# refresh-bio/DSRC

Hardware: AMD Instinct MI355X
Metric: raw FASTQ MB/s compressed (bit-identical .dsrc) at -d3 -q2 (higher is better)
Workload: dtype u8/u16/u32 integer

## Files before the change

### dsrc_amd/csrc/k_parse.h

```cpp
#pragma once
#include "k_common.h"

typedef u64 __attribute__((aligned(1))) u64_text;

__device__ __forceinline__ u32 byte_eq8(u64 w, u64 c_rep)
{
	const u64 x = w ^ c_rep;
	const u64 y = (((x & 0x7F7F7F7F7F7F7F7Full) + 0x7F7F7F7F7F7F7F7Full) | x) | 0x7F7F7F7F7F7F7F7Full;
	return (u32)((((~y) >> 7) * 0x0102040810204080ull) >> 56);
}

struct LineBits { u64 term, crlf; };

__device__ __forceinline__ LineBits classify64(const u8* p, u64 base, u64 size)
{
	LineBits r; r.term = 0; r.crlf = 0;
	if (base >= size) return r;
	u64 lf = 0, cr = 0;
	if (base + DSRC_LANE_BYTES <= size)
	{
#pragma unroll
		for (u32 k = 0; k < DSRC_LANE_BYTES / 8; ++k)
		{
			const u64 w = *(const u64_text*)(p + base + 8 * k);
			lf |= (u64)byte_eq8(w, 0x0A0A0A0A0A0A0A0Aull) << (8 * k);
			cr |= (u64)byte_eq8(w, 0x0D0D0D0D0D0D0D0Dull) << (8 * k);
		}
	}
	else
	{
		for (u32 k = 0; base + k < size; ++k)
		{
			const u8 c = p[base + k];
			if (c == '\n') lf |= 1ull << k;
			if (c == '\r') cr |= 1ull << k;
		}
	}
	const u64 n_valid = size - base;
	const u64 valid = n_valid >= 64 ? ~0ull : ((1ull << n_valid) - 1ull);
	const bool lf_next = base + DSRC_LANE_BYTES < size && p[base + DSRC_LANE_BYTES] == '\n';
	const bool cr_prev = base > 0 && p[base - 1] == '\r';
	const u64 lf_after = (lf >> 1) | (lf_next ? 1ull << 63 : 0ull);
	const u64 cr_before = (cr << 1) | (cr_prev ? 1ull : 0ull);
	r.term = (lf | (cr & ~lf_after)) & valid;
	r.crlf = (lf & cr_before) & valid;
	return r;
}

__global__ void __launch_bounds__(WG) k_count_lines(const u8* in, const BlkDesc* desc, BlkState* st, u32* tile_cnt, DsrcParams prm)
{
	__shared__ u32 s_tot[2];
	const u32 b = blockIdx.y, tile = blockIdx.x;
	const BlkDesc d = desc[b];
	if (tile >= d.n_tiles) return;
	if (threadIdx.x < 2) s_tot[threadIdx.x] = 0;
	__syncthreads();
	const LineBits lb = classify64(in + d.in_off, (u64)tile * DSRC_TILE_BYTES + (u64)threadIdx.x * DSRC_LANE_BYTES, d.in_size);
	const u32 cnt = wave_sum((u32)__popcll(lb.term)), crlf = wave_sum((u32)__popcll(lb.crlf));
	if (lane_id() == 0) { if (cnt) atomicAdd(&s_tot[0], cnt); if (crlf) atomicAdd(&s_tot[1], crlf); }
	__syncthreads();
	if (threadIdx.x == 0)
	{
		tile_cnt[(u64)b * prm.max_tiles + tile] = s_tot[0];
		atomicAdd(&st[b].n_term, s_tot[0]);
		if (s_tot[1]) atomicAdd(&st[b].n_crlf, s_tot[1]);
	}
}

__global__ void __launch_bounds__(WG) k_scan_tiles(const BlkDesc* desc, u32* tile_cnt, DsrcParams prm)
{
	const u32 b = blockIdx.x;
	const u32 n = desc[b].n_tiles;
	u32* t = tile_cnt + (u64)b * prm.max_tiles;
	u32 carry = 0;
	for (u32 base = 0; base < n; base += blockDim.x)
	{
		const u32 i = base + threadIdx.x;
		const u32 v = i < n ? t[i] : 0;
		u32 tot;
		const u32 ex = block_excl_scan(v, &tot);
		if (i < n) t[i] = carry + ex;
		carry += tot;
	}
}

__global__ void __launch_bounds__(WG) k_index_lines(const u8* in, const BlkDesc* desc, const u32* tile_base, u32* line_start, DsrcParams prm)
{
	const u32 b = blockIdx.y, tile = blockIdx.x;
	const BlkDesc d = desc[b];
	if (tile >= d.n_tiles) return;
	const u64 base = (u64)tile * DSRC_TILE_BYTES + (u64)threadIdx.x * DSRC_LANE_BYTES;
	const LineBits lb = classify64(in + d.in_off, base, d.in_size);
	u64 mask = lb.term;
	u32 total;
	u32 rank = block_excl_scan((u32)__popcll(mask), &total) + tile_base[(u64)b * prm.max_tiles + tile];
	u32* ls = line_start + d.line_base;
	if (tile == 0 && threadIdx.x == 0) ls[0] = 0;
	while (mask)
	{
		const u32 k = (u32)__ffsll((long long)mask) - 1;
		mask &= mask - 1;
		ls[++rank] = (u32)(base + k + 1) | ((u32)((lb.crlf >> k) & 1ull) << 31);
	}
}

struct RecPools
{
	u32* title_off; u32* seq_off; u32* qual_off;
	u16* title_len; u16* len;
	u16* kept; u16* trunc;
	u32* q_off; u32* d_off;
};

#define LS_POS(x) ((x) & 0x7FFFFFFFu)
__device__ __forceinline__ void line_extent(const u32* ls, u32 n_term, u32 size, u32 i, u32* start, u32* len)
{
	if (i > n_term) { *start = size; *len = 0; return; }
	const u32 s = LS_POS(ls[i]);
	*start = s;
	if (i == n_term) { *len = size - s; return; }
	const u32 nx = ls[i + 1];
	const u32 e = LS_POS(nx) - 1 - (nx >> 31);
	*len = e - s;
}

__global__ void __launch_bounds__(WG) k_records(const u8* in, const BlkDesc* desc, BlkState* st, const u32* line_start, RecPools rp)
{
	const u32 b = blockIdx.y;
	const BlkDesc d = desc[b];
	const u32 n_term = st[b].n_term;
	const u32 r = blockIdx.x * blockDim.x + threadIdx.x;
	const u32 n_cand = (n_term + 1 + 3) / 4;
	if (r >= n_cand || r >= d.rec_cap) return;
	const u8* p = in + d.in_off;
	const u32* ls = line_start + d.line_base;
	u32 s0, l0, s1, l1, s2, l2, s3, l3;
	line_extent(ls, n_term, d.in_size, 4 * r + 0, &s0, &l0);
	line_extent(ls, n_term, d.in_size, 4 * r + 1, &s1, &l1);
	line_extent(ls, n_term, d.in_size, 4 * r + 2, &s2, &l2);
	line_extent(ls, n_term, d.in_size, 4 * r + 3, &s3, &l3);
	const bool ok = s0 < d.in_size && l0 > 0 && p[s0] == '@' && l2 > 0 && l1 == l3;
	if (!ok) atomicMin(&st[b].first_bad, r);
	if (l0 > 65535u || l1 > 65535u || l3 > 65535u) atomicOr(&st[b].err, (u32)DSRC_ERR_LONG_LINE);
	const u64 g = (u64)d.rec_base + r;
	rp.title_off[g] = s0; rp.title_len[g] = (u16)l0;
	rp.seq_off[g] = s1;   rp.len[g] = (u16)l1;
	rp.qual_off[g] = s3;
}

__device__ __forceinline__ u32 dna_index(u32 c)
{
	switch (c)
	{
	case 'A': return 0; case 'G': return 1; case 'C': return 2; case 'T': return 3; case 'N': return 4;
	case 'R': return 5; case 'W': return 6; case 'S': return 7; case 'K': return 8; case 'M': return 9;
	case 'D': return 10; case 'V': return 11; case 'H': return 12; case 'B': return 13; case 'Y': return 14;
	case 'X': return 15; case 'U': return 16; case '.': return 17; case '-': return 18;
	default: return 255;
	}
}

constexpr u32 dna_index_packed(u32 c, u64 K0, u64 K1)
{
	const u32 i = c - 'A';
	const bool lo = i < 12;
	const u64 k = lo ? K0 : K1;
	const u32 j = lo ? i : i - 12;
	const u32 sh = 5 * (j < 12 ? j : 12);
	u32 v = i < 25 ? (u32)(k >> sh) & 31u : 31u;
	v = c == '.' ? 17u : v;
	v = c == '-' ? 18u : v;
	return v == 31u ? 255u : v;
}
#define DNA_INDEX_K0 0x0fa3ff607ff509a0ull
#define DNA_INDEX_K1 0xe7997019cbfffc89ull
constexpr u32 dna_index_switch_c(u32 c)
{
	switch (c)
	{
	case 'A': return 0; case 'G': return 1; case 'C': return 2; case 'T': return 3; case 'N': return 4;
	case 'R': return 5; case 'W': return 6; case 'S': return 7; case 'K': return 8; case 'M': return 9;
	case 'D': return 10; case 'V': return 11; case 'H': return 12; case 'B': return 13; case 'Y': return 14;
	case 'X': return 15; case 'U': return 16; case '.': return 17; case '-': return 18;
	default: return 255;
	}
}
constexpr bool dna_index_same()
{
	for (u32 c = 0; c < 256; ++c) if (dna_index_packed(c, DNA_INDEX_K0, DNA_INDEX_K1) != dna_index_switch_c(c)) return false;
	return true;
}
static_assert(dna_index_same(), "dna_index: packed table differs from src/RecordsProcessor.cpp:186-206");
template <bool FAST> __device__ __forceinline__ u32 dna_index_t(u32 c) { return FAST ? dna_index_packed(c, DNA_INDEX_K0, DNA_INDEX_K1) : dna_index(c); }

__device__ __forceinline__ u32 lossy_bin(u32 q)
{
	if (q < 2) return 0; if (q < 10) return 1; if (q < 20) return 2; if (q < 25) return 3;
	if (q < 30) return 4; if (q < 35) return 5; if (q < 40) return 6; if (q < 64) return 7;
	return 255;
}

#ifndef FAST_STATS
#define FAST_STATS true
#endif
#ifndef FAST_WRITE
#define FAST_WRITE true
#endif
__device__ __forceinline__ u32 transform_base_s(u32 s, u32 qual, u32 qoff, u32 lossy, u32* sidx, bool* keep);
template <bool FAST = false>
__device__ __forceinline__ u32 transform_base(u32 base, u32 qual, u32 qoff, u32 lossy, u32* sidx, bool* keep)
{
	return transform_base_s(dna_index_t<FAST>(base), qual, qoff, lossy, sidx, keep);
}
__device__ __forceinline__ void dna_index_table(u8* lut) { for (u32 i = threadIdx.x; i < 256; i += blockDim.x) lut[i] = (u8)dna_index(i); }
__device__ __forceinline__ u32 transform_base_s(u32 s, u32 qual, u32 qoff, u32 lossy, u32* sidx, bool* keep)
{
	*sidx = s;
	u32 q;
	if (!lossy)
	{
		q = (qual - qoff) & 255u;
		if (s > 3 && q < 7) { q = (q + 128u + ((s - 2u) << 3) - 16u) & 255u; *keep = false; }
		else *keep = true;
	}
	else
	{
		q = lossy_bin((qual - qoff) & 255u);
		if (s >= 4) { q = 0; *keep = false; }
		else { if (q == 0) q = 1; *keep = true; }
	}
	return q;
}

__device__ __forceinline__ u32 block_rec_count(const BlkState& S, const BlkDesc& d)
{
	u32 n_cand = (S.n_term + 1 + 3) / 4;
	if (n_cand > d.rec_cap) n_cand = d.rec_cap;
	return S.first_bad < n_cand ? S.first_bad : n_cand;
}

__global__ void __launch_bounds__(64) k_rec_count(const BlkDesc* desc, BlkState* st, u32 n_blocks)
{
	const u32 b = blockIdx.x * blockDim.x + threadIdx.x;
	if (b < n_blocks) st[b].n_recs = block_rec_count(st[b], desc[b]);
}

__device__ __forceinline__ u32 cs_state(u32 c) { return c == 'C' ? 1u : c == 'G' ? 2u : c == 'T' ? 3u : 0u; }

__global__ void __launch_bounds__(WG) k_cs_decode(u8* in, const BlkDesc* desc, BlkState* st, RecPools rp)
{
	const u32 b = blockIdx.y;
	const BlkDesc d = desc[b];
	u8* p = in + d.in_off;
	const u32 n_recs = st[b].n_recs;
	const u32 lane = lane_id();
	const u32 waves_total = gridDim.x * (blockDim.x >> 6);
	for (u32 r = blockIdx.x * (blockDim.x >> 6) + wave_id(); r < n_recs; r += waves_total)
	{
		const u64 g = (u64)d.rec_base + r;
		const u32 len = rp.len[g], so = rp.seq_off[g];
		if (len == 0) continue;
		if (lane == 0 && p[so] != p[rp.seq_off[d.rec_base]]) atomicOr(&st[b].cs_varbegin, 1u);
		u32 state = cs_state(p[so]);
		bool bad = false;
		for (u32 j0 = 0; j0 < len; j0 += 64)
		{
			const u32 j = j0 + lane;
			const bool in_r = j < len && j >= 1;
			const u32 c = in_r ? (u32)p[so + j] - '.' : 0u;
			if (c > 5) bad = true;
			const u32 col = (in_r && c >= 2 && c <= 5) ? c - 2 : 0u;
			const u64 m0 = __ballot((col & 1u) != 0), m1 = __ballot((col & 2u) != 0);
			const u64 le = lanemask_lt() | (1ull << lane);
			const u32 mine = state ^ ((u32)__popcll(m0 & le) & 1u) ^ (((u32)__popcll(m1 & le) & 1u) << 1);
			if (in_r) p[so + j] = c < 2 ? (u8)'N' : (u8)"ACGT"[mine];
			state ^= ((u32)__popcll(m0) & 1u) ^ (((u32)__popcll(m1) & 1u) << 1);
		}
		if (bad) atomicOr(&st[b].err, (u32)DSRC_ERR_BAD_BASE);
	}
}

#define STATS_PARTS_SLOT 7
__global__ void __launch_bounds__(WG) k_prep_stats(const u8* in, const BlkDesc* desc, BlkState* st, RecPools rp, DsrcParams prm)
{
	__shared__ u32 s_qf[256];
	__shared__ u32 s_df[20];
	__shared__ u32 s_acc[8];
	__shared__ u8 s_dna[256];
	__shared__ u32 s_last;
	dna_index_table(s_dna);
	const u32 b = blockIdx.y, parts = gridDim.x;
	const BlkDesc d = desc[b];
	const u8* p = in + d.in_off;
	const u32 n_recs = block_rec_count(st[b], d);

	for (u32 i = threadIdx.x; i < 256; i += blockDim.x) s_qf[i] = 0;
	if (threadIdx.x < 20) s_df[threadIdx.x] = 0;
	if (threadIdx.x < 8) s_acc[threadIdx.x] = (threadIdx.x == 3) ? 0xFFFFFFFFu : 0u;
	__syncthreads();

	const u32 lane = lane_id();
	u32 a_rle = 0, a_th = 0, a_raw = 0, a_min = 0xFFFFFFFFu, a_max = 0, a_tag = 0, a_bad = 0;
	constexpr u32 PS_AHEAD = 3;
	const u32 wstep = (blockDim.x >> 6) * parts, w0 = blockIdx.x * (blockDim.x >> 6) + wave_id();
	u32 n_len = 0, n_so = 0, n_qo = 0, n_tl = 0, n_b[PS_AHEAD], n_q[PS_AHEAD];
#pragma unroll
	for (u32 k = 0; k < PS_AHEAD; ++k) { n_b[k] = 'A'; n_q[k] = 0; }
	auto request = [&](u64 g)
	{
		n_len = rp.len[g]; n_so = rp.seq_off[g]; n_qo = rp.qual_off[g]; n_tl = rp.title_len[g];
		const u32 last = n_len ? n_len - 1u : 0u;
#pragma unroll
		for (u32 k = 0; k < PS_AHEAD; ++k)
		{
			const u32 j = min_u32(64u * k + lane, last);
			n_b[k] = p[n_so + j]; n_q[k] = p[n_qo + j];
		}
	};
	if (w0 < n_recs) request((u64)d.rec_base + w0);
	for (u32 r = w0; r < n_recs; r += wstep)
	{
		const u64 g = (u64)d.rec_base + r;
		const u32 len = n_len, so = n_so, qo = n_qo, tl = n_tl;
		u32 c_b[PS_AHEAD], c_q[PS_AHEAD];
#pragma unroll
		for (u32 k = 0; k < PS_AHEAD; ++k) { c_b[k] = n_b[k]; c_q[k] = n_q[k]; }
		if (r + wstep < n_recs) request(g + wstep);
		u32 kept = 0, th = 0, rle = 0, carry = 255, lastq = 255;
		auto chunk = [&](const u32 j0, const u32 cb_in, const u32 cq_in)
		{
			const u32 j = j0 + lane;
			const bool in_r = j < len;
			u32 sidx = 0, q = 0; bool keep = false;
			{
				const u32 cb = in_r ? cb_in : (u32)'A', cq = in_r ? cq_in : prm.quality_offset + 40u;
				const u32 qq = transform_base_s((u32)s_dna[cb & 255u], cq, prm.quality_offset, prm.lossy, &sidx, &keep);
				if (in_r) q = qq; else { keep = false; sidx = 0; }
			}
			const bool k2 = in_r && keep;
			if (in_r && sidx >= 20) a_bad = 1;
			if (k2 && sidx < 20) atomicAdd(&s_df[sidx], 1u);
			kept += (u32)__popcll(__ballot(k2));
			const u32 prev = wave_shr1(q, carry);
			const u64 change = __ballot(in_r && q != prev);
			rle += (u32)__popcll(change);
			if (__popcll(change) <= 16)
			{
				const u64 starts = change | 1ull;
				const u64 after = (starts >> lane) >> 1;
				const u32 n_in = len - j0 < 64u ? len - j0 : 64u;
				const u32 run = after ? (u32)__ffsll((long long)after) : n_in - lane;
				if (in_r && ((starts >> lane) & 1ull)) atomicAdd(&s_qf[q], run);
			}
			else if (in_r) atomicAdd(&s_qf[q], 1u);
			const u64 m2 = __ballot(in_r && q != 2);
			if (m2) th = j0 + 63u - (u32)__clzll((long long)m2);
			carry = (u32)__builtin_amdgcn_readlane((int)q, 63);
			const u32 last_lane = (len - 1 - j0) < 64u ? (len - 1 - j0) : 63u;
			lastq = (u32)__builtin_amdgcn_readlane((int)q, (int)last_lane);
		};
#pragma unroll
		for (u32 k = 0; k < PS_AHEAD; ++k) if (64u * k < len) chunk(64u * k, c_b[k], c_q[k]);
		for (u32 j0 = 64u * PS_AHEAD; j0 < len; j0 += 64)
		{
			const u32 j = min_u32(j0 + lane, len - 1u);
			chunk(j0, (u32)p[so + j], (u32)p[qo + j]);
		}
		if (len > 0 && lastq == 2 && rle > 0) rle -= 1;
		if (lane == 0)
		{
			rp.kept[g] = (u16)kept;
			rp.trunc[g] = (u16)(th + (len > 0 ? 1u : 0u));
			a_rle += rle; a_th += th; a_raw += len; a_tag += tl;
			a_min = len < a_min ? len : a_min; a_max = len > a_max ? len : a_max;
		}
	}
	if (lane == 0)
	{
		atomicAdd(&s_acc[0], a_rle); atomicAdd(&s_acc[1], a_th); atomicAdd(&s_acc[2], a_raw);
		atomicMin(&s_acc[3], a_min); atomicMax(&s_acc[4], a_max); atomicAdd(&s_acc[5], a_tag);
	}
	if (a_bad) atomicOr(&s_acc[7], 1u);
	__syncthreads();

	BlkState* S = &st[b];
	if (parts > 1)
	{
		for (u32 i = threadIdx.x; i < 256; i += blockDim.x) if (s_qf[i]) atomicAdd(&S->q_freq[i], s_qf[i]);
		if (threadIdx.x < 20 && s_df[threadIdx.x]) atomicAdd(&S->d_freq[threadIdx.x], s_df[threadIdx.x]);
		if (threadIdx.x == 0)
		{
			atomicAdd(&S->rle_len, s_acc[0]); atomicAdd(&S->th_len, s_acc[1]); atomicAdd(&S->raw_len, s_acc[2]);
			atomicMin(&S->min_len, s_acc[3]); atomicMax(&S->max_len, s_acc[4]); atomicAdd(&S->raw_tag, s_acc[5]);
			if (s_acc[7]) atomicOr(&S->err, (u32)DSRC_ERR_BAD_BASE);
		}
		__threadfence();
		__syncthreads();
		if (threadIdx.x == 0) s_last = atomicAdd(&S->scratch[STATS_PARTS_SLOT], 1u) == parts - 1u ? 1u : 0u;
		__syncthreads();
		if (!s_last) return;
		__threadfence();
		for (u32 i = threadIdx.x; i < 256; i += blockDim.x) s_qf[i] = atomicAdd(&S->q_freq[i], 0u);
		if (threadIdx.x < 20) s_df[threadIdx.x] = atomicAdd(&S->d_freq[threadIdx.x], 0u);
		if (threadIdx.x == 0)
		{
			s_acc[0] = atomicAdd(&S->rle_len, 0u); s_acc[1] = atomicAdd(&S->th_len, 0u); s_acc[2] = atomicAdd(&S->raw_len, 0u);
			s_acc[3] = atomicAdd(&S->min_len, 0u); s_acc[4] = atomicAdd(&S->max_len, 0u); s_acc[5] = atomicAdd(&S->raw_tag, 0u);
			s_acc[7] = 0;
			S->scratch[STATS_PARTS_SLOT] = 0;
		}
		__syncthreads();
	}
	else
	{
		for (u32 i = threadIdx.x; i < 256; i += blockDim.x) S->q_freq[i] = s_qf[i];
		if (threadIdx.x < 20) S->d_freq[threadIdx.x] = s_df[threadIdx.x];
	}
	if (threadIdx.x == 0)
	{
		S->n_recs = n_recs;
		S->n_lines = S->n_term + 1;
		S->rle_len = s_acc[0]; S->th_len = s_acc[1]; S->raw_len = s_acc[2];
		S->min_len = s_acc[3]; S->max_len = s_acc[4];
		S->raw_tag = s_acc[5]; S->raw_dna = s_acc[2]; S->raw_qua = s_acc[2];
		u32 e = 0;
		if (n_recs == 0) e |= DSRC_ERR_NO_RECORDS;
		if (s_acc[7]) e |= DSRC_ERR_BAD_BASE;
		if (e) atomicOr(&S->err, e);
		u32 dc = 0, qc = 0;
		for (u32 i = 0; i < 20; ++i) S->d_sym[i] = s_df[i] ? (u8)dc++ : (u8)255;
		for (u32 i = 0; i < 256; ++i) S->q_sym[i] = s_qf[i] ? (u8)qc++ : (u8)255;
		S->d_count = dc; S->q_count = qc;
	}
}

__global__ void __launch_bounds__(WG) k_cs_reduce(const u8* in, const BlkDesc* desc, BlkState* st, RecPools rp, DsrcParams prm)
{
	const u32 b = blockIdx.y;
	BlkState* S = &st[b];
	if (S->cs_varbegin) return;
	const BlkDesc d = desc[b];
	const u32 r = blockIdx.x * blockDim.x + threadIdx.x;
	if (r >= S->n_recs) return;
	const u64 g = (u64)d.rec_base + r;
	const u32 len = rp.len[g];
	if (r == 0)
	{
		const u8* p = in + d.in_off;
		u32 first = 255, q0 = 0;
		for (u32 j = 0; j < len && first == 255; ++j)
		{
			u32 sidx; bool keep;
			const u32 q = transform_base(p[rp.seq_off[g] + j], p[rp.qual_off[g] + j], prm.quality_offset, prm.lossy, &sidx, &keep);
			if (j == 0) q0 = q;
			if (keep) first = sidx;
		}
		S->cs_seq_begin = first != 255 ? first : (len ? dna_index(p[rp.seq_off[g]]) : 0u);
		S->cs_qua_begin = q0;
		S->cs_reduced = 1;
	}
	if (rp.kept[g] < 1 || len < 2) { atomicOr(&S->err, (u32)DSRC_ERR_BAD_BASE); return; }
	rp.len[g] = (u16)(len - 1); rp.qual_off[g] += 1; rp.kept[g] -= 1;
	if (rp.trunc[g] > 0) rp.trunc[g] -= 1;
}

__global__ void __launch_bounds__(WG) k_rec_offsets(const BlkDesc* desc, BlkState* st, RecPools rp)
{
	const u32 b = blockIdx.x;
	const BlkDesc d = desc[b];
	const u32 n = st[b].n_recs;
	u32 cq = 0, cd = 0;
	for (u32 base = 0; base < n; base += blockDim.x)
	{
		const u32 r = base + threadIdx.x;
		const u64 g = (u64)d.rec_base + r;
		const u32 vq = r < n ? rp.len[g] : 0, vd = r < n ? rp.kept[g] : 0;
		u32 tq, td;
		const u32 eq = block_excl_scan(vq, &tq);
		const u32 ed = block_excl_scan(vd, &td);
		if (r < n) { rp.q_off[g] = cq + eq; rp.d_off[g] = cd + ed; }
		cq += tq; cd += td;
	}
	if (threadIdx.x == 0) { st[b].q_total = cq; st[b].d_total = cd; }
}

__global__ void __launch_bounds__(WG) k_prep_write(const u8* in, const BlkDesc* desc, const BlkState* st, RecPools rp,
												   u8* q_stream, u8* qp_stream, u8* d_stream, DsrcParams prm)
{
	__shared__ u8 s_dna[256];
	dna_index_table(s_dna);
	__syncthreads();
	const u32 b = blockIdx.y;
	const BlkDesc d = desc[b];
	const u8* p = in + d.in_off;
	const u32 n_recs = st[b].n_recs;
	const u32 lane = lane_id();
	const bool write_qp = st[b].min_len != st[b].max_len;
	const u32 red = st[b].cs_reduced;
	const u32 waves_total = gridDim.x * (blockDim.x >> 6);
	constexpr u32 PW_AHEAD = 3;
	u32 n_rlen = 0, n_so = 0, n_qo = 0, n_qoff = 0, n_doff = 0;
	auto request = [&](u64 g) { n_rlen = rp.len[g]; n_so = rp.seq_off[g]; n_qo = rp.qual_off[g]; n_qoff = rp.q_off[g]; n_doff = rp.d_off[g]; };
	const u32 r0 = blockIdx.x * (blockDim.x >> 6) + wave_id();
	if (r0 < n_recs) request((u64)d.rec_base + r0);
	for (u32 r = r0; r < n_recs; r += waves_total)
	{
		const u64 g = (u64)d.rec_base + r;
		const u32 rlen = n_rlen, len = rlen + red, so = n_so, qo = n_qo - red;
		u8* qs = q_stream + d.q_base + n_qoff;
		u8* qps = qp_stream + d.q_base + n_qoff;
		u8* ds = d_stream + d.d_base + n_doff;
		u32 c_b[PW_AHEAD], c_q[PW_AHEAD];
#pragma unroll
		for (u32 k = 0; k < PW_AHEAD; ++k)
		{
			const u32 j = min_u32(64u * k + lane, len ? len - 1u : 0u);
			c_b[k] = p[so + j]; c_q[k] = p[qo + j];
		}
		if (r + waves_total < n_recs) request(g + waves_total);
		u32 run = 0;
		auto chunk = [&](const u32 j0, const u32 cb_in, const u32 cq_in)
		{
			const u32 j = j0 + lane;
			const bool in_r = j < len;
			u32 sidx = 0, q = 0; bool keep = false;
			{
				const u32 cb = in_r ? cb_in : (u32)'A', cq = in_r ? cq_in : prm.quality_offset + 40u;
				const u32 qq = transform_base_s((u32)s_dna[cb & 255u], cq, prm.quality_offset, prm.lossy, &sidx, &keep);
				if (in_r) q = qq; else { keep = false; sidx = 0; }
			}
			const bool k2 = in_r && keep;
			const u64 km = __ballot(k2);
			if (in_r && j >= red) { qs[j - red] = (u8)q; if (write_qp) qps[j - red] = (u8)(((j - red) * 128u) / rlen); }
			const u32 at = run + (u32)__popcll(km & lanemask_lt());
			if (k2 && at >= red) ds[at - red] = (u8)sidx;
			run += (u32)__popcll(km);
		};
#pragma unroll
		for (u32 k = 0; k < PW_AHEAD; ++k) if (64u * k < len) chunk(64u * k, c_b[k], c_q[k]);
		for (u32 j0 = 64u * PW_AHEAD; j0 < len; j0 += 64)
		{
			const u32 j = min_u32(j0 + lane, len - 1u);
			chunk(j0, (u32)p[so + j], (u32)p[qo + j]);
		}
	}
}
```

Before: 65860.

## Process four records per wave with 16-lane groups using SWAR byte ops in prep

Adds a lossless fast path for the prep stats and prep write kernels. Each wave now handles four records at once, each lane covering 16 bytes through packed 64-bit bitwise tricks: ACGT coding, quality subtraction, run detection and DPP group scans. This replaces the old one-record-per-wave loop with per-byte lanes and many shared atomics. Records longer than 256 bytes, reduced-checksum blocks and lossy mode fall back to the old path, and stats also gains a launch-bounds occupancy hint, at the cost of considerably more code complexity.

```diff
diff --git a/dsrc_amd/csrc/k_parse.h b/dsrc_amd/csrc/k_parse.h
--- a/dsrc_amd/csrc/k_parse.h
+++ b/dsrc_amd/csrc/k_parse.h
@@ -280,8 +280,45 @@
 	}
 }
 
+struct PsRec { u32 kept, th, rle, carry, lastq; };
+__device__ __forceinline__ void ps_chunk(PsRec& R, u32& a_bad, const u32 j0, const u32 cb_in, const u32 cq_in, const u32 len,
+										 const DsrcParams& prm, const u8* s_dna, u32* s_df, u32* s_qf)
+{
+	const u32 lane = lane_id(), j = j0 + lane;
+	const bool in_r = j < len;
+	u32 sidx = 0, q = 0; bool keep = false;
+	{
+		const u32 cb = in_r ? cb_in : (u32)'A', cq = in_r ? cq_in : prm.quality_offset + 40u;
+		const u32 qq = transform_base_s((u32)s_dna[cb & 255u], cq, prm.quality_offset, prm.lossy, &sidx, &keep);
+		if (in_r) q = qq; else { keep = false; sidx = 0; }
+	}
+	const bool k2 = in_r && keep;
+	if (in_r && sidx >= 20) a_bad = 1;
+	if (k2 && sidx < 20) atomicAdd(&s_df[sidx], 1u);
+	R.kept += (u32)__popcll(__ballot(k2));
+	const u32 prev = wave_shr1(q, R.carry);
+	const u64 change = __ballot(in_r && q != prev);
+	R.rle += (u32)__popcll(change);
+	if (__popcll(change) <= 16)
+	{
+		const u64 starts = change | 1ull;
+		const u64 after = (starts >> lane) >> 1;
+		const u32 n_in = len - j0 < 64u ? len - j0 : 64u;
+		const u32 run = after ? (u32)__ffsll((long long)after) : n_in - lane;
+		if (in_r && ((starts >> lane) & 1ull)) atomicAdd(&s_qf[q], run);
+	}
+	else if (in_r) atomicAdd(&s_qf[q], 1u);
+	const u64 m2 = __ballot(in_r && q != 2);
+	if (m2) R.th = j0 + 63u - (u32)__clzll((long long)m2);
+	R.carry = (u32)__builtin_amdgcn_readlane((int)q, 63);
+	const u32 last_lane = (len - 1 - j0) < 64u ? (len - 1 - j0) : 63u;
+	R.lastq = (u32)__builtin_amdgcn_readlane((int)q, (int)last_lane);
+}
+
+#include "k_prep.h"
+
 #define STATS_PARTS_SLOT 7
-__global__ void __launch_bounds__(WG) k_prep_stats(const u8* in, const BlkDesc* desc, BlkState* st, RecPools rp, DsrcParams prm)
+__global__ void __launch_bounds__(WG, 8) k_prep_stats(const u8* in, const BlkDesc* desc, BlkState* st, RecPools rp, DsrcParams prm)
 {
 	__shared__ u32 s_qf[256];
 	__shared__ u32 s_df[20];
@@ -301,81 +338,55 @@
 
 	const u32 lane = lane_id();
 	u32 a_rle = 0, a_th = 0, a_raw = 0, a_min = 0xFFFFFFFFu, a_max = 0, a_tag = 0, a_bad = 0;
-	constexpr u32 PS_AHEAD = 3;
-	const u32 wstep = (blockDim.x >> 6) * parts, w0 = blockIdx.x * (blockDim.x >> 6) + wave_id();
-	u32 n_len = 0, n_so = 0, n_qo = 0, n_tl = 0, n_b[PS_AHEAD], n_q[PS_AHEAD];
-#pragma unroll
-	for (u32 k = 0; k < PS_AHEAD; ++k) { n_b[k] = 'A'; n_q[k] = 0; }
-	auto request = [&](u64 g)
-	{
-		n_len = rp.len[g]; n_so = rp.seq_off[g]; n_qo = rp.qual_off[g]; n_tl = rp.title_len[g];
-		const u32 last = n_len ? n_len - 1u : 0u;
-#pragma unroll
-		for (u32 k = 0; k < PS_AHEAD; ++k)
-		{
-			const u32 j = min_u32(64u * k + lane, last);
-			n_b[k] = p[n_so + j]; n_q[k] = p[n_qo + j];
-		}
-	};
-	if (w0 < n_recs) request((u64)d.rec_base + w0);
-	for (u32 r = w0; r < n_recs; r += wstep)
-	{
-		const u64 g = (u64)d.rec_base + r;
-		const u32 len = n_len, so = n_so, qo = n_qo, tl = n_tl;
-		u32 c_b[PS_AHEAD], c_q[PS_AHEAD];
-#pragma unroll
-		for (u32 k = 0; k < PS_AHEAD; ++k) { c_b[k] = n_b[k]; c_q[k] = n_q[k]; }
-		if (r + wstep < n_recs) request(g + wstep);
-		u32 kept = 0, th = 0, rle = 0, carry = 255, lastq = 255;
-		auto chunk = [&](const u32 j0, const u32 cb_in, const u32 cq_in)
-		{
-			const u32 j = j0 + lane;
-			const bool in_r = j < len;
-			u32 sidx = 0, q = 0; bool keep = false;
+	const bool groups = !prm.lossy && d.in_size >= 16u;
+	if (groups) prep_stats_groups(p, d, n_recs, rp, prm, s_dna, s_df, s_qf, &s_acc[7], a_rle, a_th, a_raw, a_min, a_max, a_tag, a_bad);
+	else
+	{
+		constexpr u32 PS_AHEAD = 3;
+		const u32 wstep = (blockDim.x >> 6) * parts, w0 = blockIdx.x * (blockDim.x >> 6) + wave_id();
+		u32 n_len = 0, n_so = 0, n_qo = 0, n_tl = 0, n_b[PS_AHEAD], n_q[PS_AHEAD];
+#pragma unroll
+		for (u32 k = 0; k < PS_AHEAD; ++k) { n_b[k] = 'A'; n_q[k] = 0; }
+		auto request = [&](u64 g)
+		{
+			n_len = rp.len[g]; n_so = rp.seq_off[g]; n_qo = rp.qual_off[g]; n_tl = rp.title_len[g];
+			const u32 last = n_len ? n_len - 1u : 0u;
+#pragma unroll
+			for (u32 k = 0; k < PS_AHEAD; ++k)
 			{
-				const u32 cb = in_r ? cb_in : (u32)'A', cq = in_r ? cq_in : prm.quality_offset + 40u;
-				const u32 qq = transform_base_s((u32)s_dna[cb & 255u], cq, prm.quality_offset, prm.lossy, &sidx, &keep);
-				if (in_r) q = qq; else { keep = false; sidx = 0; }
+				const u32 j = min_u32(64u * k + lane, last);
+				n_b[k] = p[n_so + j]; n_q[k] = p[n_qo + j];
 			}
-			const bool k2 = in_r && keep;
-			if (in_r && sidx >= 20) a_bad = 1;
-			if (k2 && sidx < 20) atomicAdd(&s_df[sidx], 1u);
-			kept += (u32)__popcll(__ballot(k2));
-			const u32 prev = wave_shr1(q, carry);
-			const u64 change = __ballot(in_r && q != prev);
-			rle += (u32)__popcll(change);
-			if (__popcll(change) <= 16)
+		};
+		if (w0 < n_recs) request((u64)d.rec_base + w0);
+		for (u32 r = w0; r < n_recs; r += wstep)
+		{
+			const u64 g = (u64)d.rec_base + r;
+			const u32 len = n_len, so = n_so, qo = n_qo, tl = n_tl;
+			u32 c_b[PS_AHEAD], c_q[PS_AHEAD];
+#pragma unroll
+			for (u32 k = 0; k < PS_AHEAD; ++k) { c_b[k] = n_b[k]; c_q[k] = n_q[k]; }
+			if (r + wstep < n_recs) request(g + wstep);
+			PsRec R = { 0, 0, 0, 255, 255 };
+			auto chunk = [&](const u32 j0, const u32 cb_in, const u32 cq_in) { ps_chunk(R, a_bad, j0, cb_in, cq_in, len, prm, s_dna, s_df, s_qf); };
+#pragma unroll
+			for (u32 k = 0; k < PS_AHEAD; ++k) if (64u * k < len) chunk(64u * k, c_b[k], c_q[k]);
+			for (u32 j0 = 64u * PS_AHEAD; j0 < len; j0 += 64)
 			{
-				const u64 starts = change | 1ull;
-				const u64 after = (starts >> lane) >> 1;
-				const u32 n_in = len - j0 < 64u ? len - j0 : 64u;
-				const u32 run = after ? (u32)__ffsll((long long)after) : n_in - lane;
-				if (in_r && ((starts >> lane) & 1ull)) atomicAdd(&s_qf[q], run);
+				const u32 j = min_u32(j0 + lane, len - 1u);
+				chunk(j0, (u32)p[so + j], (u32)p[qo + j]);
 			}
-			else if (in_r) atomicAdd(&s_qf[q], 1u);
-			const u64 m2 = __ballot(in_r && q != 2);
-			if (m2) th = j0 + 63u - (u32)__clzll((long long)m2);
-			carry = (u32)__builtin_amdgcn_readlane((int)q, 63);
-			const u32 last_lane = (len - 1 - j0) < 64u ? (len - 1 - j0) : 63u;
-			lastq = (u32)__builtin_amdgcn_readlane((int)q, (int)last_lane);
-		};
-#pragma unroll
-		for (u32 k = 0; k < PS_AHEAD; ++k) if (64u * k < len) chunk(64u * k, c_b[k], c_q[k]);
-		for (u32 j0 = 64u * PS_AHEAD; j0 < len; j0 += 64)
-		{
-			const u32 j = min_u32(j0 + lane, len - 1u);
-			chunk(j0, (u32)p[so + j], (u32)p[qo + j]);
-		}
-		if (len > 0 && lastq == 2 && rle > 0) rle -= 1;
-		if (lane == 0)
-		{
-			rp.kept[g] = (u16)kept;
-			rp.trunc[g] = (u16)(th + (len > 0 ? 1u : 0u));
-			a_rle += rle; a_th += th; a_raw += len; a_tag += tl;
-			a_min = len < a_min ? len : a_min; a_max = len > a_max ? len : a_max;
-		}
-	}
-	if (lane == 0)
+			if (len > 0 && R.lastq == 2 && R.rle > 0) R.rle -= 1;
+			if (lane == 0)
+			{
+				rp.kept[g] = (u16)R.kept;
+				rp.trunc[g] = (u16)(R.th + (len > 0 ? 1u : 0u));
+				a_rle += R.rle; a_th += R.th; a_raw += len; a_tag += tl;
+				a_min = len < a_min ? len : a_min; a_max = len > a_max ? len : a_max;
+			}
+		}
+	}
+	if (lane == 0 || groups)
 	{
 		atomicAdd(&s_acc[0], a_rle); atomicAdd(&s_acc[1], a_th); atomicAdd(&s_acc[2], a_raw);
 		atomicMin(&s_acc[3], a_min); atomicMax(&s_acc[4], a_max); atomicAdd(&s_acc[5], a_tag);
@@ -497,51 +508,56 @@
 	const u32 lane = lane_id();
 	const bool write_qp = st[b].min_len != st[b].max_len;
 	const u32 red = st[b].cs_reduced;
-	const u32 waves_total = gridDim.x * (blockDim.x >> 6);
-	constexpr u32 PW_AHEAD = 3;
-	u32 n_rlen = 0, n_so = 0, n_qo = 0, n_qoff = 0, n_doff = 0;
-	auto request = [&](u64 g) { n_rlen = rp.len[g]; n_so = rp.seq_off[g]; n_qo = rp.qual_off[g]; n_qoff = rp.q_off[g]; n_doff = rp.d_off[g]; };
-	const u32 r0 = blockIdx.x * (blockDim.x >> 6) + wave_id();
-	if (r0 < n_recs) request((u64)d.rec_base + r0);
-	for (u32 r = r0; r < n_recs; r += waves_total)
-	{
-		const u64 g = (u64)d.rec_base + r;
-		const u32 rlen = n_rlen, len = rlen + red, so = n_so, qo = n_qo - red;
-		u8* qs = q_stream + d.q_base + n_qoff;
-		u8* qps = qp_stream + d.q_base + n_qoff;
-		u8* ds = d_stream + d.d_base + n_doff;
-		u32 c_b[PW_AHEAD], c_q[PW_AHEAD];
-#pragma unroll
-		for (u32 k = 0; k < PW_AHEAD; ++k)
-		{
-			const u32 j = min_u32(64u * k + lane, len ? len - 1u : 0u);
-			c_b[k] = p[so + j]; c_q[k] = p[qo + j];
-		}
-		if (r + waves_total < n_recs) request(g + waves_total);
-		u32 run = 0;
-		auto chunk = [&](const u32 j0, const u32 cb_in, const u32 cq_in)
-		{
-			const u32 j = j0 + lane;
-			const bool in_r = j < len;
-			u32 sidx = 0, q = 0; bool keep = false;
+	if (!prm.lossy && !red && st[b].max_len <= PG_SPAN && d.in_size >= 16u)
+		prep_write_groups(p, d, n_recs, rp, q_stream + d.q_base, qp_stream + d.q_base, d_stream + d.d_base, write_qp, prm, s_dna);
+	else
+	{
+		const u32 waves_total = gridDim.x * (blockDim.x >> 6);
+		constexpr u32 PW_AHEAD = 3;
+		u32 n_rlen = 0, n_so = 0, n_qo = 0, n_qoff = 0, n_doff = 0;
+		auto request = [&](u64 g) { n_rlen = rp.len[g]; n_so = rp.seq_off[g]; n_qo = rp.qual_off[g]; n_qoff = rp.q_off[g]; n_doff = rp.d_off[g]; };
+		const u32 r0 = blockIdx.x * (blockDim.x >> 6) + wave_id();
+		if (r0 < n_recs) request((u64)d.rec_base + r0);
+		for (u32 r = r0; r < n_recs; r += waves_total)
+		{
+			const u64 g = (u64)d.rec_base + r;
+			const u32 rlen = n_rlen, len = rlen + red, so = n_so, qo = n_qo - red;
+			u8* qs = q_stream + d.q_base + n_qoff;
+			u8* qps = qp_stream + d.q_base + n_qoff;
+			u8* ds = d_stream + d.d_base + n_doff;
+			u32 c_b[PW_AHEAD], c_q[PW_AHEAD];
+#pragma unroll
+			for (u32 k = 0; k < PW_AHEAD; ++k)
 			{
-				const u32 cb = in_r ? cb_in : (u32)'A', cq = in_r ? cq_in : prm.quality_offset + 40u;
-				const u32 qq = transform_base_s((u32)s_dna[cb & 255u], cq, prm.quality_offset, prm.lossy, &sidx, &keep);
-				if (in_r) q = qq; else { keep = false; sidx = 0; }
+				const u32 j = min_u32(64u * k + lane, len ? len - 1u : 0u);
+				c_b[k] = p[so + j]; c_q[k] = p[qo + j];
 			}
-			const bool k2 = in_r && keep;
-			const u64 km = __ballot(k2);
-			if (in_r && j >= red) { qs[j - red] = (u8)q; if (write_qp) qps[j - red] = (u8)(((j - red) * 128u) / rlen); }
-			const u32 at = run + (u32)__popcll(km & lanemask_lt());
-			if (k2 && at >= red) ds[at - red] = (u8)sidx;
-			run += (u32)__popcll(km);
-		};
-#pragma unroll
-		for (u32 k = 0; k < PW_AHEAD; ++k) if (64u * k < len) chunk(64u * k, c_b[k], c_q[k]);
-		for (u32 j0 = 64u * PW_AHEAD; j0 < len; j0 += 64)
-		{
-			const u32 j = min_u32(j0 + lane, len - 1u);
-			chunk(j0, (u32)p[so + j], (u32)p[qo + j]);
-		}
-	}
-}
+			if (r + waves_total < n_recs) request(g + waves_total);
+			u32 run = 0;
+			auto chunk = [&](const u32 j0, const u32 cb_in, const u32 cq_in)
+			{
+				const u32 j = j0 + lane;
+				const bool in_r = j < len;
+				u32 sidx = 0, q = 0; bool keep = false;
+				{
+					const u32 cb = in_r ? cb_in : (u32)'A', cq = in_r ? cq_in : prm.quality_offset + 40u;
+					const u32 qq = transform_base_s((u32)s_dna[cb & 255u], cq, prm.quality_offset, prm.lossy, &sidx, &keep);
+					if (in_r) q = qq; else { keep = false; sidx = 0; }
+				}
+				const bool k2 = in_r && keep;
+				const u64 km = __ballot(k2);
+				if (in_r && j >= red) { qs[j - red] = (u8)q; if (write_qp) qps[j - red] = (u8)(((j - red) * 128u) / rlen); }
+				const u32 at = run + (u32)__popcll(km & lanemask_lt());
+				if (k2 && at >= red) ds[at - red] = (u8)sidx;
+				run += (u32)__popcll(km);
+			};
+#pragma unroll
+			for (u32 k = 0; k < PW_AHEAD; ++k) if (64u * k < len) chunk(64u * k, c_b[k], c_q[k]);
+			for (u32 j0 = 64u * PW_AHEAD; j0 < len; j0 += 64)
+			{
+				const u32 j = min_u32(j0 + lane, len - 1u);
+				chunk(j0, (u32)p[so + j], (u32)p[qo + j]);
+			}
+		}
+	}
+}
diff --git a/dsrc_amd/csrc/k_prep.h b/dsrc_amd/csrc/k_prep.h
--- /dev/null
+++ b/dsrc_amd/csrc/k_prep.h
@@ -0,0 +1,320 @@
+#pragma once
+
+#define PG_SPAN 256u
+#define B8(x) (0x0101010101010101ull * (u64)(x))
+
+typedef u32 __attribute__((aligned(1))) u32_text;
+typedef u16 __attribute__((aligned(1))) u16_text;
+
+struct W16 { u64 lo, hi; };
+
+constexpr u64 nz_bytes(u64 x) { return (((x & B8(0x7F)) + B8(0x7F)) | x) & B8(0x80); }
+constexpr u64 sub_bytes(u64 x, u64 y_low7, u64 y_not) { return ((x | B8(0x80)) - y_low7) ^ ((x ^ y_not) & B8(0x80)); }
+constexpr u64 acgt_code(u64 c) { return ((c >> 2) & B8(1)) | ((((c >> 1) ^ (c >> 2)) & B8(1)) << 1); }
+constexpr u64 acgt_miss(u64 c)
+{
+	const u64 t = (c >> 2) & ~(c >> 1) & B8(1);
+	return (c & B8(0xF9)) ^ B8(0x41) ^ (t | (t << 4));
+}
+constexpr bool acgt_words_same()
+{
+	for (u32 c = 0; c < 256; ++c)
+		for (u32 at = 0; at < 64; at += 8)
+		{
+			const u64 w = (B8(0x41) & ~(0xFFull << at)) | ((u64)c << at);
+			const u32 s = dna_index_switch_c(c);
+			const u64 miss = acgt_miss(w), code = acgt_code(w);
+			if ((miss & ~(0xFFull << at)) != 0 || (code & ~(0xFFull << at)) != 0) return false;
+			if (s <= 3 ? (((miss >> at) & 255u) != 0 || ((code >> at) & 255u) != s) : ((miss >> at) & 255u) == 0) return false;
+		}
+	return true;
+}
+static_assert(acgt_words_same(), "acgt_code / acgt_miss differ from dna_index");
+
+__device__ __forceinline__ u32 pack8(u64 m)
+{
+	u32 a = (u32)(m >> 7) & 0x01010101u, b = (u32)(m >> 39) & 0x01010101u;
+	a |= a >> 7; a |= a >> 14; b |= b >> 7; b |= b >> 14;
+	return (a & 15u) | ((b & 15u) << 4);
+}
+__device__ __forceinline__ u32 pack16(W16 m) { return pack8(m.lo) | (pack8(m.hi) << 8); }
+__device__ __forceinline__ u64 low_bytes(u32 n) { return n >= 8 ? ~0ull : (1ull << (8 * n)) - 1ull; }
+
+__device__ __forceinline__ u32 get_byte(W16 w, u32 i) { return (u32)(((i & 8u) ? w.hi : w.lo) >> (8 * (i & 7u))) & 255u; }
+__device__ __forceinline__ void set_byte(W16& w, u32 i, u32 v)
+{
+	const u32 sh = 8 * (i & 7u);
+	const u64 m = 0xFFull << sh, nv = (u64)v << sh;
+	if (i & 8u) w.hi = (w.hi & ~m) | nv; else w.lo = (w.lo & ~m) | nv;
+}
+__device__ __forceinline__ void del_byte(W16& w, u32 i)
+{
+	const u64 m = (1ull << (8 * (i & 7u))) - 1ull;
+	if (i & 8u) w.hi = (w.hi & m) | ((w.hi >> 8) & ~m);
+	else { w.lo = (w.lo & m) | (((w.lo >> 8) | (w.hi << 56)) & ~m); w.hi >>= 8; }
+}
+__device__ __forceinline__ W16 shr_bytes(W16 w, u32 n)
+{
+	if (n >= 16) { w.lo = 0; w.hi = 0; return w; }
+	if (n & 8u) { w.lo = w.hi; w.hi = 0; }
+	const u32 sh = 8 * (n & 7u);
+	if (sh) { w.lo = (w.lo >> sh) | (w.hi << (64 - sh)); w.hi >>= sh; }
+	return w;
+}
+
+__device__ __forceinline__ W16 text_load(const u8* p, u32 at, u32 top)
+{
+	const u8* a = p + min_u32(at, top);
+	W16 w; w.lo = *(const u64_text*)a; w.hi = *(const u64_text*)(a + 8);
+	return w;
+}
+__device__ __forceinline__ u32 text_held_back(u32 at, u32 top) { return at - min_u32(at, top); }
+
+__device__ __forceinline__ void store_bytes(u8* p, W16 w, u32 n)
+{
+	if (n >= 16) { *(u64_text*)p = w.lo; *(u64_text*)(p + 8) = w.hi; return; }
+	u64 v = w.lo;
+	if (n & 8u) { *(u64_text*)p = v; v = w.hi; p += 8; }
+	if (n & 4u) { *(u32_text*)p = (u32)v; v >>= 32; p += 4; }
+	if (n & 2u) { *(u16_text*)p = (u16)v; v >>= 16; p += 2; }
+	if (n & 1u) *p = (u8)v;
+}
+
+__device__ __forceinline__ u32 group_shr1(u32 v, u32 first)
+{
+#ifdef DSRC_EMU_BUILD
+	const u32 t = __shfl_up(v, 1);
+	return (lane_id() & 15u) == 0 ? first : t;
+#else
+	return (u32)__builtin_amdgcn_update_dpp((int)first, (int)v, 0x111, 0xf, 0xf, false);
+#endif
+}
+__device__ __forceinline__ u32 group_incl_scan(u32 v)
+{
+#ifdef DSRC_EMU_BUILD
+	for (u32 d = 1; d < 16; d <<= 1)
+	{
+		const u32 t = __shfl_up(v, d);
+		if ((lane_id() & 15u) >= d) v += t;
+	}
+	return v;
+#else
+	int x = (int)v;
+	x += __builtin_amdgcn_update_dpp(0, x, 0x111, 0xf, 0xf, false);
+	x += __builtin_amdgcn_update_dpp(0, x, 0x112, 0xf, 0xf, false);
+	x += __builtin_amdgcn_update_dpp(0, x, 0x114, 0xf, 0xf, false);
+	x += __builtin_amdgcn_update_dpp(0, x, 0x118, 0xf, 0xf, false);
+	return (u32)x;
+#endif
+}
+__device__ __forceinline__ u32 group_bits(u64 ballot)
+{
+	const u32 half = (lane_id() & 32u) ? (u32)(ballot >> 32) : (u32)ballot;
+	return (half >> (lane_id() & 16u)) & 0xFFFFu;
+}
+
+struct GroupLane
+{
+	W16 b, q;
+	W16 in;
+	u32 n;
+	u32 other;
+};
+__device__ __forceinline__ GroupLane group_lane(W16 wb, W16 wq, u32 held_b, u32 held_q, u32 len, u32 g, u32 qoff)
+{
+	GroupLane L;
+	if (__ballot((held_b | held_q) != 0)) { wb = shr_bytes(wb, held_b); wq = shr_bytes(wq, held_q); }
+	L.n = len > 16u * g ? min_u32(len - 16u * g, 16u) : 0u;
+	L.in.lo = low_bytes(L.n); L.in.hi = low_bytes(L.n > 8u ? L.n - 8u : 0u);
+	const u64 y_low7 = B8(qoff & 0x7Fu), y_not = ~B8(qoff & 255u);
+	L.b = wb;
+	L.q.lo = sub_bytes(wq.lo, y_low7, y_not); L.q.hi = sub_bytes(wq.hi, y_low7, y_not);
+	W16 miss; miss.lo = acgt_miss(wb.lo) & L.in.lo; miss.hi = acgt_miss(wb.hi) & L.in.hi;
+	L.other = 0;
+	if ((miss.lo | miss.hi) != 0) { miss.lo = nz_bytes(miss.lo); miss.hi = nz_bytes(miss.hi); L.other = pack16(miss); }
+	return L;
+}
+__device__ __forceinline__ u32 hoisted_quality(u32 q, u32 s) { return (q + 128u + ((s - 2u) << 3) - 16u) & 255u; }
+
+template <typename T> __device__ __forceinline__ T& pool_at(T* base, u32 i) { return *(T*)((u8*)base + (size_t)(u32)(i * (u32)sizeof(T))); }
+struct BlockPools
+{
+	const u32* seq_off; const u32* qual_off; const u16* title_len; const u16* len; u16* kept; u16* trunc; const u32* q_off; const u32* d_off;
+	__device__ __forceinline__ BlockPools(const RecPools& rp, u32 rec_base)
+		: seq_off(rp.seq_off + rec_base), qual_off(rp.qual_off + rec_base), title_len(rp.title_len + rec_base), len(rp.len + rec_base),
+		  kept(rp.kept + rec_base), trunc(rp.trunc + rec_base), q_off(rp.q_off + rec_base), d_off(rp.d_off + rec_base) {}
+};
+
+__device__ __forceinline__ void prep_stats_groups(const u8* p, const BlkDesc& d, const u32 n_recs, RecPools rp, const DsrcParams& prm,
+												  const u8* s_dna, u32* s_df, u32* s_qf, u32* s_bad,
+												  u32& a_rle, u32& a_th, u32& a_raw, u32& a_min, u32& a_max, u32& a_tag, u32& a_bad)
+{
+	const u32 lane = lane_id(), g = lane & 15u, gi = lane >> 4;
+	const u32 step = (blockDim.x >> 6) * gridDim.x * 4u, rb0 = (blockIdx.x * (blockDim.x >> 6) + wave_id()) * 4u;
+	const u32 top = d.in_size - 16u;
+	const BlockPools bp(rp, d.rec_base);
+	u32 n_ok = 0, n_b1 = 0, n_b2 = 0, n_b12 = 0;
+	u32 n_len = 0, n_so = 0, n_qo = 0;
+	W16 n_wb = { 0, 0 }, n_wq = { 0, 0 };
+	auto request = [&](u32 rb)
+	{
+		const u32 r = min_u32(rb + gi, n_recs - 1u);
+		n_len = pool_at(bp.len, r); n_so = pool_at(bp.seq_off, r); n_qo = pool_at(bp.qual_off, r);
+		n_wb = text_load(p, n_so + 16u * g, top); n_wq = text_load(p, n_qo + 16u * g, top);
+	};
+	bool any_over = false;
+	if (rb0 < n_recs) request(rb0);
+	for (u32 rb = rb0; rb < n_recs; rb += step)
+	{
+		const bool have = rb + gi < n_recs;
+		const u32 len = n_len, so = n_so, qo = n_qo;
+		const W16 wb = n_wb, wq = n_wq;
+		const bool mine = have && len <= PG_SPAN;
+		GroupLane L = group_lane(wb, wq, text_held_back(so + 16u * g, top), text_held_back(qo + 16u * g, top), mine ? len : 0u, g, prm.quality_offset);
+
+		{
+			const u64 o0 = L.in.lo & B8(1), o1 = L.in.hi & B8(1);
+			const u64 x0 = (L.b.lo >> 1) & o0, x1 = (L.b.hi >> 1) & o1, y0 = (L.b.lo >> 2) & o0, y1 = (L.b.hi >> 2) & o1;
+			n_ok += L.n;
+			n_b1 += (u32)__popcll(x0) + (u32)__popcll(x1);
+			n_b2 += (u32)__popcll(y0) + (u32)__popcll(y1);
+			n_b12 += (u32)__popcll(x0 & y0) + (u32)__popcll(x1 & y1);
+		}
+		u32 left = 0;
+		for (u32 m = L.other; m; m &= m - 1u)
+		{
+			const u32 i = (u32)__ffs((int)m) - 1u;
+			const u32 c = get_byte(L.b, i), q = get_byte(L.q, i);
+			const u32 s = s_dna[c];
+			n_ok -= 1; n_b1 -= (c >> 1) & 1u; n_b2 -= (c >> 2) & 1u; n_b12 -= (c >> 1) & (c >> 2) & 1u;
+			if (s >= 20) atomicOr(s_bad, 1u);
+			if (q < 7) { set_byte(L.q, i, hoisted_quality(q, s)); ++left; }
+			else if (s < 20) atomicAdd(&s_df[s], 1u);
+		}
+		const u64 leave = __ballot(left != 0);
+		u32 left_to_here = 0;
+		if (leave) left_to_here = group_incl_scan(left);
+		if (mine && g == 15u) pool_at(bp.kept, rb + gi) = (u16)(len - left_to_here);
+
+		const u32 front = group_shr1((u32)(L.q.hi >> 56), 255u);
+		W16 ch;
+		ch.lo = nz_bytes(L.q.lo ^ ((L.q.lo << 8) | front)) & L.in.lo;
+		ch.hi = nz_bytes(L.q.hi ^ ((L.q.hi << 8) | (L.q.lo >> 56))) & L.in.hi;
+		const u32 n_ch = (u32)__popcll(ch.lo) + (u32)__popcll(ch.hi);
+		a_rle += n_ch;
+		const u32 rec_ch = group_bits(__ballot(n_ch != 0));
+		if (mine && len > 0 && g == ((len - 1u) >> 4) && get_byte(L.q, (len - 1u) & 15u) == 2 && rec_ch != 0) a_rle -= 1;
+
+		W16 n2;
+		n2.lo = nz_bytes(L.q.lo ^ B8(2)) & L.in.lo; n2.hi = nz_bytes(L.q.hi ^ B8(2)) & L.in.hi;
+		const u32 rec_n2 = group_bits(__ballot((n2.lo | n2.hi) != 0));
+		const u32 g_n2 = rec_n2 ? 31u - (u32)__clz((int)rec_n2) : 0u;
+		if (mine && g == g_n2)
+		{
+			const u32 at = n2.hi ? 8u + ((63u - (u32)__clzll((long long)n2.hi)) >> 3) : ((63u - (u32)__clzll((long long)n2.lo)) >> 3);
+			const u32 th = rec_n2 ? 16u * g + at : 0u;
+			pool_at(bp.trunc, rb + gi) = (u16)(th + (len > 0 ? 1u : 0u));
+			a_th += th;
+		}
+		if (rb + step < n_recs) request(rb + step);
+
+		for (u32 starts = (pack16(ch) | 1u) & ((1u << L.n) - 1u); starts; )
+		{
+			const u32 i = (u32)__ffs((int)starts) - 1u;
+			starts &= starts - 1u;
+			const u32 end = starts ? (u32)__ffs((int)starts) - 1u : L.n;
+			atomicAdd(&s_qf[get_byte(L.q, i)], end - i);
+		}
+
+		any_over |= __ballot(have && len > PG_SPAN) != 0;
+	}
+	if (any_over)
+		for (u32 rb = rb0; rb < n_recs; rb += step)
+		{
+			const u32 r = min_u32(rb + gi, n_recs - 1u);
+			for (u64 over = __ballot(rb + gi < n_recs && g == 0 && pool_at(bp.len, r) > PG_SPAN); over; over &= over - 1ull)
+			{
+				const u32 ro = rb + (((u32)__ffsll((long long)over) - 1u) >> 4);
+				const u32 o_len = pool_at(bp.len, ro), o_so = pool_at(bp.seq_off, ro), o_qo = pool_at(bp.qual_off, ro);
+				PsRec R = { 0, 0, 0, 255, 255 };
+				for (u32 j0 = 0; j0 < o_len; j0 += 64)
+				{
+					const u32 j = min_u32(j0 + lane, o_len - 1u);
+					ps_chunk(R, a_bad, j0, (u32)p[o_so + j], (u32)p[o_qo + j], o_len, prm, s_dna, s_df, s_qf);
+				}
+				if (R.lastq == 2 && R.rle > 0) R.rle -= 1;
+				if (lane == 0)
+				{
+					pool_at(bp.kept, ro) = (u16)R.kept;
+					pool_at(bp.trunc, ro) = (u16)(R.th + 1u);
+					a_rle += R.rle; a_th += R.th;
+				}
+			}
+		}
+	for (u32 r = blockIdx.x * blockDim.x + threadIdx.x; r < n_recs; r += blockDim.x * gridDim.x)
+	{
+		const u32 len = pool_at(bp.len, r);
+		a_raw += len; a_tag += pool_at(bp.title_len, r);
+		a_min = len < a_min ? len : a_min; a_max = len > a_max ? len : a_max;
+	}
+	const u32 c_g = n_b12, c_c = n_b1 - n_b12, c_t = n_b2 - n_b12, c_a = n_ok - n_b1 - n_b2 + n_b12;
+	if (c_a) atomicAdd(&s_df[0], c_a);
+	if (c_g) atomicAdd(&s_df[1], c_g);
+	if (c_c) atomicAdd(&s_df[2], c_c);
+	if (c_t) atomicAdd(&s_df[3], c_t);
+}
+
+__device__ __forceinline__ void prep_write_groups(const u8* p, const BlkDesc& d, const u32 n_recs, RecPools rp, u8* qs, u8* qps, u8* ds,
+												  const bool write_qp, const DsrcParams& prm, const u8* s_dna)
+{
+	const u32 lane = lane_id(), g = lane & 15u, gi = lane >> 4;
+	const u32 step = (blockDim.x >> 6) * gridDim.x * 4u, rb0 = (blockIdx.x * (blockDim.x >> 6) + wave_id()) * 4u;
+	const u32 top = d.in_size - 16u;
+	const BlockPools bp(rp, d.rec_base);
+	u32 n_len = 0, n_so = 0, n_qo = 0, n_qoff = 0, n_doff = 0;
+	W16 n_wb = { 0, 0 }, n_wq = { 0, 0 };
+	auto request = [&](u32 rb)
+	{
+		const u32 r = min_u32(rb + gi, n_recs - 1u);
+		n_len = pool_at(bp.len, r); n_so = pool_at(bp.seq_off, r); n_qo = pool_at(bp.qual_off, r); n_qoff = pool_at(bp.q_off, r); n_doff = pool_at(bp.d_off, r);
+		n_wb = text_load(p, n_so + 16u * g, top); n_wq = text_load(p, n_qo + 16u * g, top);
+	};
+	if (rb0 < n_recs) request(rb0);
+	for (u32 rb = rb0; rb < n_recs; rb += step)
+	{
+		const bool have = rb + gi < n_recs;
+		const u32 len = n_len, so = n_so, qo = n_qo, qoff = n_qoff, doff = n_doff;
+		const W16 wb = n_wb, wq = n_wq;
+		if (rb + step < n_recs) request(rb + step);
+		GroupLane L = group_lane(wb, wq, text_held_back(so + 16u * g, top), text_held_back(qo + 16u * g, top), have ? len : 0u, g, prm.quality_offset);
+		W16 sy; sy.lo = acgt_code(L.b.lo); sy.hi = acgt_code(L.b.hi);
+		u32 left = 0;
+		for (u32 m = L.other; m; )
+		{
+			const u32 i = 31u - (u32)__clz((int)m);
+			m ^= 1u << i;
+			const u32 s = s_dna[get_byte(L.b, i)], q = get_byte(L.q, i);
+			if (q < 7) { set_byte(L.q, i, hoisted_quality(q, s)); del_byte(sy, i); ++left; }
+			else set_byte(sy, i, s);
+		}
+		store_bytes(qs + qoff + 16u * g, L.q, L.n);
+		if (write_qp)
+		{
+			const u32 dv = len ? len : 1u;
+			const u32 inc = 128u / dv, inc_r = 128u % dv;
+			u32 x = (16u * g * 128u) / dv, r = (16u * g * 128u) % dv;
+			W16 c = { 0, 0 };
+#pragma unroll
+			for (u32 i = 0; i < 16; ++i)
+			{
+				if (i < 8) c.lo |= (u64)(x & 255u) << (8 * i); else c.hi |= (u64)(x & 255u) << (8 * (i - 8));
+				x += inc; r += inc_r;
+				if (r >= dv) { r -= dv; ++x; }
+			}
+			store_bytes(qps + qoff + 16u * g, c, L.n);
+		}
+		u32 below = 16u * g;
+		if (__ballot(left != 0)) below -= group_incl_scan(left) - left;
+		store_bytes(ds + doff + below, sy, L.n - left);
+	}
+}
```

Result: faster. 69240, median of 6 (+5.1%).
